# inhavl-shlee/AFI-GAN

Hardware: AMD Instinct MI355X
Metric: stage1_G+D_step_images_per_s (higher is better)
Workload: dtype f32 via f16x3: two scaled fp16 pieces per operand, three f16 MFMAs per product, fp32 accumulate (tensors fp32)

## Files before the change

### afigan_amd/csrc/afi_launch.h

```cpp
#pragma once
#include "afi_common.h"

int afi_launch_pix_gemm(const AfiPixGemm& p, int b_rc, hipStream_t st);
int afi_launch_gemm_tn(const float* Q, const float* V, float* dU, int planes, long long rows_per_plane, int M, int N, hipStream_t st, bool deterministic = false);
int afi_launch_gemm_nt(const float* A, const float* B, float* C, int planes, long long rows_per_plane, int N, int K, hipStream_t st);
int afi_launch_split_bf16_tiles(const float* B, void* out, int planes, int N, int K, int split, hipStream_t st);
int afi_launch_gemm_nt_bf16_dma(const float* A, const void* Bsplit, float* C, int planes, long long rows_per_plane, int N, int K, int split, hipStream_t st);
int afi_launch_gemm_tn_bf16(const float* Q, const float* V, float* dU, int planes, long long rows_per_plane, int M, int N, int split, hipStream_t st, bool deterministic = false);
int afi_launch_split_f16_tiles(const float* B, void* out, int planes, int N, int K, hipStream_t st, int wkind = 0);
int afi_f16_image_begin(void* out, hipStream_t st);
float* afi_f16_image_wmax(void* out);
long long afi_f16_image_bytes(int planes, int N, int K);
int afi_launch_absmax_planes(const float* X, long long per_plane, int planes, float* out, hipStream_t st);
AfiF16Bound afi_f16_bound(const float* amax, int kind);
int afi_launch_gemm_nt_f16x3(const float* A, const void* Bimg, float* C, int planes, long long rows_per_plane, int N, int K, const AfiF16Bound& ab, hipStream_t st,
                             bool a_pre = false, long long nt256_min_tiles = 512, bool local_sums = false);
int afi_launch_gemm_tn_f16x3(const float* Q, const float* V, float* dU, int planes, long long rows_per_plane, int M, int N, const AfiF16Bound& qb, const AfiF16Bound& vb,
                             hipStream_t st, bool pre = false, bool deterministic = false);
int afi_launch_wgrad_gemm(const AfiWgradGemm& p, hipStream_t st);
int afi_launch_wgrad_gemm_group(const AfiWgradGemm* probs, int n, int wide, hipStream_t st);
int afi_launch_wgrad_gemm_group6(const AfiWgradGemm* probs, int n, hipStream_t st);
int afi_launch_pix_gemm_group(const AfiPixGemm* probs, int n, int b_rc, hipStream_t st);

long long afi_wk6_image_bytes(int Ncols, int Ck, int ntaps, int nKphase);
int afi_launch_wk6_images(const AfiWk6ImgJob* jobs, int n, hipStream_t st, const AfiWk6Side* side = nullptr, const AfiWk6ConvT* ct = nullptr);
int afi_launch_pix_gemm_sk(const AfiPixGemm& p, int b_rc, hipStream_t st);
int afi_launch_pix_gemm_wk_group(const AfiPixGemm* probs, int n, int b_rc, hipStream_t st);
int afi_launch_wgrad_group(const AfiWgradGemm* probs, int n, int wide, hipStream_t st);
int afi_launch_wgrad6_group(const AfiWgradGemm* probs, int n, hipStream_t st);

int afi_launch_nchw_to_nhwc(const float* in, float* out, int N, int C, int P, hipStream_t st);
int afi_launch_cast_to_f32_nhwc(const void* in, int dt, int N, int C, int H, int W, long long sN, long long sC, long long sH, long long sW, float* out,
                                hipStream_t st);
int afi_launch_cast_from_f32_nhwc(const AfiView& in, int N, int H, int W, int C, void* out, int dt, hipStream_t st);

int afi_launch_colsum_group(const AfiColsumProb* probs, int n, hipStream_t st);
int afi_launch_nhwc_to_nchw(const float* in, float* out, int N, int C, int P, hipStream_t st);
int afi_launch_convT_pack(const float* W, float* Wp, int Cin, int Cout, hipStream_t st);
int afi_launch_convT_unpack_grad(const float* dWp, float* dW, int Cin, int Cout, hipStream_t st);
int afi_launch_rdb_wgrad_unpack(const float* dWp, float* const dw[4], int C, int G, float alpha, hipStream_t st);
int afi_launch_rdb_wgrad_unpack_multi(const float* dWp, long long stride, float* const (*dw)[4], int nblocks, int C, int G, float alpha, hipStream_t st);
int afi_launch_g_bwd_tail(const AfiColsumProb* cs, int n_cs, const float* dWpT, float* dWT, int Cin, int Cout,
                          const float* dWp, long long stride, float* const (*dw)[4], int nblocks, int C, int G, float alpha, hipStream_t st);
int afi_launch_rdb_xpart_pack(const float* const w[4], float* out, int C, int G, hipStream_t st);
int afi_launch_lrelu_slice(AfiView v, int N, int H, int W, int nch, hipStream_t st);
int afi_launch_bn_stats(const float* x, long long P, int C, float* mean, float* invstd, float* var_out, float* running_mean,
                        float* running_var, float* scratch, hipStream_t st, long long* num_batches_tracked = nullptr, float eps = -1.f,
                        float momentum = -1.f, bool fp64 = true);
int afi_launch_bn_stats_from_partials(const double* partial, int rows, long long P, int C, float* mean, float* invstd, float* var_out, float* running_mean,
                                      float* running_var, hipStream_t st, long long* num_batches_tracked = nullptr, float eps = -1.f, float momentum = -1.f);
int afi_launch_view_absmax(AfiView x, int N, int H, int W, int C, float* amax, hipStream_t st);
int afi_launch_bn_apply_lrelu(const float* x, float* y, const float* mean, const float* invstd, const float* gamma, const float* beta,
// ... 50 lines not shown
```

### afigan_amd/csrc/igemm.hip

```cpp
#include "afi_common.h"
#include "afi_launch.h"

#define AFI_BK 32
#define AFI_LDK (AFI_BK + 4)


__device__ __attribute__((aligned(16))) float afi_zeros[4] = {0.f, 0.f, 0.f, 0.f};

#include "afi_epilogue.h"

template <bool POST>
__global__ __launch_bounds__(256) void afi_pix_splitk_epilogue_kernel(const AfiPixGemm p) {
    const int HW = p.H * p.W;
    const long long M = (long long)p.N * HW;
    const int ldp = (p.Ncols + 3) & ~3;
    const int C_F4 = ldp >> 2;
    const long long total = M * C_F4;
    for (long long it = (long long)blockIdx.x * 256 + threadIdx.x; it < total; it += (long long)gridDim.x * 256) {
        const long long m = it / C_F4;
        const int col = (int)(it - m * C_F4) * 4;
        f32x4 v = {0.f, 0.f, 0.f, 0.f};
        const float* src = p.partial + m * ldp + col;
        const long long slab = M * ldp;
        int ks = 0;
// ... 509 lines not shown
#include <mutex>
namespace {
struct ProfRec { hipEvent_t a, b; int kind; double flops; long long m; int n, k, split, planes; };
struct ProfState {
    std::atomic<bool> on{false};
    std::mutex mu;
    std::vector<ProfRec> recs;
    std::vector<hipEvent_t> pool;
    size_t used = 0;
} g_prof;
const char* kKindNames[] = {
    "pix_gemm<128x128,KC,linear> (1x1 / ragged-map / non-aligned Winograd GEMMs)", "pix_gemm<128x64,KC>", "pix_gemm<128x32,KC>", "pix_gemm<64x64,KC>",
    "pix_gemm<128x128,RC,linear> (conv dgrad, mid-size / ragged maps)", "pix_gemm<128x64,RC>", "pix_gemm<128x32,RC>", "pix_gemm<64x64,RC>",
    "wgrad_gemm<128x128>", "wgrad_gemm<64x128>", "wgrad_gemm<32x128>",
    "pix_gemm<128x128,KC,halo> (conv fwd)", "pix_gemm<128x128,RC,halo> (conv dgrad)",
    "gemm_nt<128x128> (batched Winograd GEMM)", "gemm_tn<128x128> (Winograd weight-gradient GEMM)",
    "pix_gemm_wk (small-map pixel GEMM, K split inside the block; grouped launches included)",
    "wgrad_group (grouped weight gradients of a small-map backward pass)",
    "gemm_nt_bf16<128x128> (batched Winograd GEMM on the bf16 MFMA: bf16x6 / bf16x3 / bf16 operands, fp32 accumulate)",
    "gemm_tn_bf16<128x128> (Winograd weight-gradient GEMM on the bf16 MFMA: bf16x6 / bf16x3 / bf16 operands, fp32 accumulate)",
    "wgrad_group6 (grouped weight gradients of a small-map backward pass on the bf16 MFMA, bf16x6 operands, fp32 accumulate)",
    "pix_gemm_wk6 (small-map pixel GEMM on the bf16 MFMA, bf16x6 operands on pre-split weight images, fp32 accumulate; grouped launches included)",
    "gemm_nt_f16x3 (batched Winograd GEMM on the f16 MFMA, 256x256 tiles where the grid fills the chip and 128x128 below: two scaled fp16 pieces per operand, three products, fp32 accumulate)",
    "gemm_tn_f16x3<128x128> (Winograd weight-gradient GEMM on the f16 MFMA: two scaled fp16 pieces per operand, three products, fp32 accumulate)"};
constexpr int kNumKinds = 23;
hipEvent_t prof_event() {
    if (g_prof.used == g_prof.pool.size()) {
        hipEvent_t e;
        (void)hipEventCreate(&e);
        g_prof.pool.push_back(e);
    }
    return g_prof.pool[g_prof.used++];
}
struct ProfScope {
    hipStream_t st; int kind; double flops; hipEvent_t a{};
    long long m = 0; int n = 0, k = 0, split = 1, planes = 1;
    ProfScope(hipStream_t s, int kd, double f) : st(s), kind(kd), flops(f) {
        if (g_prof.on) { std::lock_guard<std::mutex> lk(g_prof.mu); a = prof_event(); (void)hipEventRecord(a, st); started = true; }
    }
    bool live = true, started = false;
    void cancel() { live = false; }
    ~ProfScope() {
        if (started && live) { std::lock_guard<std::mutex> lk(g_prof.mu); hipEvent_t b = prof_event(); (void)hipEventRecord(b, st); g_prof.recs.push_back({a, b, kind, flops, m, n, k, split, planes}); }
    }
};
}

extern "C" int afi_profile_enable(int on) {
    std::lock_guard<std::mutex> lk(g_prof.mu);
    if (on) { g_prof.recs.clear(); g_prof.used = 0; }
    g_prof.on = on != 0;
    return AFI_OK;
}
extern "C" int afi_profile_num_kinds(void) { return kNumKinds; }
extern "C" const char* afi_profile_kind_name(int kind) { return (kind >= 0 && kind < kNumKinds) ? kKindNames[kind] : ""; }
extern "C" int afi_profile_get(int kind, double* out) {
    out[0] = out[1] = out[2] = 0.0;
    for (const ProfRec& r : g_prof.recs) {
        if (r.kind != kind) continue;
        if (hipEventSynchronize(r.b) != hipSuccess) return AFI_ERR_LAUNCH;
        float ms = 0.f;
        if (hipEventElapsedTime(&ms, r.a, r.b) != hipSuccess) return AFI_ERR_LAUNCH;
        out[0] += 1.0; out[1] += ms; out[2] += r.flops;
    }
    return AFI_OK;
}

#include <stdio.h>
extern "C" int afi_profile_dump(const char* path) {
// ... 441 lines not shown
```

### afigan_amd/frozen.py

```python
import torch
import torch.nn as nn

from . import ops
from ._lib import AfiError

FROZEN_BN_EPS = 1e-5


class FrozenBatchNorm2d(nn.Module):

    def __init__(self, num_features, eps=FROZEN_BN_EPS):
        super().__init__()
        self.num_features, self.eps = num_features, eps
        self.register_buffer("weight", torch.ones(num_features))
        self.register_buffer("bias", torch.zeros(num_features))
        self.register_buffer("running_mean", torch.zeros(num_features))
        self.register_buffer("running_var", torch.ones(num_features) - eps)


def fold_conv(conv, norm=None, scale=1.0):
    w = conv.weight.detach().double()
    b = conv.bias.detach().double() if conv.bias is not None else torch.zeros(w.shape[0], dtype=torch.float64, device=w.device)
    if norm is not None:
        s = norm.weight.double() * torch.rsqrt(norm.running_var.double() + norm.eps)
# ... 2 lines not shown
    w, b = w.float(), (b * scale).float().contiguous()
    k = conv.kernel_size if isinstance(conv.kernel_size, int) else (conv.kernel_size[0] if len(set(conv.kernel_size)) == 1 else 0)
    if k == 1:
        return w.reshape(w.shape[0], w.shape[1]).contiguous(), b
    if k == 3:
        return ops.to_ohwi(w), b
    return w.contiguous(), b


class Conv2d(nn.Module):

    def __init__(self, cin, cout, k, stride=1, bias=False, norm=True):
        super().__init__()
        self.kernel_size, self.stride = k, stride
        w = torch.randn(cout, cin, k, k) * (2.0 / (cout * k * k)) ** 0.5
        self.weight = nn.Parameter(w, requires_grad=False)
        self.bias = nn.Parameter(torch.zeros(cout), requires_grad=False) if bias else None
        self.norm = FrozenBatchNorm2d(cout) if norm else None

    def fold(self, scale=1.0):
        return fold_conv(self, self.norm, scale)


def conv1x1(x, wb, stride=1, add=None, relu=False, alpha=1.0, add_scale=1.0):
    if stride != 1:
        x = x[:, :, ::stride, ::stride]
    if add is not None and add.shape[-2:] != x.shape[-2:]:
        raise AfiError(f"resnet_guide: addend {tuple(add.shape)} does not match the conv output {tuple(x.shape[-2:])}")
    return ops.conv1x1_fwd(x, wb[0], wb[1], add=add, add_scale=add_scale, alpha=alpha, act=2 if relu else 0)


def conv3x3(x, wb, stride=1, relu=False):
    act = 2 if relu else 0
    if stride == 2:
        return ops.conv3x3s2_fwd(x, wb[0], wb[1], act=act)
    N, C, H, W = x.shape
    if C >= 128 and wb[0].shape[0] >= 128 and N * H * W >= 1024:
        return ops.conv3x3_wino_infer(x, wb[0], wb[1], act=act)
    return ops.conv3x3_fwd(x, wb[0], wb[1], lrelu=act)


def prepared(module, name, tensors, build):
    key = tuple((t._version, t.data_ptr(), str(t.device)) for t in tensors)
    if getattr(module, f"_{name}_key", None) != key:
        setattr(module, f"_{name}", build())
        setattr(module, f"_{name}_key", key)
    return getattr(module, f"_{name}")


def adopt_prepared(module, name, tensors):
    if not hasattr(module, f"_{name}_key"):
        raise AfiError(f"adopt_prepared: {type(module).__name__} has no prepared slot {name!r} to adopt (prepared() builds it first)")
# ... 20 lines not shown
```

### afigan_amd/guide.py

```python
import math

import torch
import torch.nn as nn
import torch.nn.functional as F

from . import ops


def _kaiming(shape, fan_in, gain=1.0):
    return torch.randn(shape) * (gain * math.sqrt(2.0 / fan_in))


class _Conv1x1(nn.Module):
    def __init__(self, cin, cout, stride=1, relu=False, gain=1.0):
        super().__init__()
        self.stride, self.relu = stride, relu
        self.register_buffer("w", _kaiming((cin, cout), cin, gain).t().contiguous())
        self.register_buffer("b", torch.zeros(cout))

    def forward(self, x, add=None, relu=None):
        if self.stride != 1:
            x = x[:, :, ::self.stride, ::self.stride]
        return ops.conv1x1_fwd(x, self.w, self.b, add=add, act=2 if (self.relu if relu is None else relu) else 0)


class _Conv3x3(nn.Module):
    def __init__(self, cin, cout, relu=False):
        super().__init__()
        self.relu = relu
        self.register_buffer("w", _kaiming((cout, 3, 3, cin), cin * 9).permute(0, 3, 1, 2))
        self.register_buffer("b", torch.zeros(cout))

    def forward(self, x):
        N, C, H, W = x.shape
        if C >= 128 and self.w.shape[0] >= 128 and N * H * W >= 1024:
            return ops.conv3x3_wino_infer(x, self.w, self.b, act=2 if self.relu else 0)
        return ops.conv3x3_fwd(x, self.w, self.b, lrelu=2 if self.relu else 0)


class _Bottleneck(nn.Module):
    def __init__(self, cin, mid, cout, stride):
        super().__init__()
        self.c1 = _Conv1x1(cin, mid, stride, relu=True)
        self.c2 = _Conv3x3(mid, mid, relu=True)
        self.c3 = _Conv1x1(mid, cout, gain=0.25)
        self.short = _Conv1x1(cin, cout, stride) if (cin != cout or stride != 1) else None
# ... 6 lines not shown
class GuideR50FPN(nn.Module):

    def __init__(self, out_channels=256):
        super().__init__()
        self.register_buffer("stem_w", _kaiming((3 * 49, 64), 3 * 49))
        self.register_buffer("stem_b", torch.zeros(64))
        cfg = [(64, 64, 256, 3, 1), (256, 128, 512, 4, 2), (512, 256, 1024, 6, 2), (1024, 512, 2048, 3, 2)]
        self.stages = nn.ModuleList()
        for cin, mid, cout, n, stride in cfg:
            blocks = [_Bottleneck(cin, mid, cout, stride)] + [_Bottleneck(cout, mid, cout, 1) for _ in range(n - 1)]
            self.stages.append(nn.Sequential(*blocks))
        self.lateral = nn.ModuleList([_Conv1x1(c, out_channels, gain=0.1) for c in (256, 512, 1024, 2048)])
        self.output = nn.ModuleList([_Conv3x3(out_channels, out_channels) for _ in range(4)])
        self.register_buffer("pixel_mean", torch.tensor([103.53, 116.28, 123.675]).view(1, 3, 1, 1))
        self.eval()

    @torch.no_grad()
    def forward(self, images):
        x = (images - self.pixel_mean) * (1.0 / 58.0)
        H, W = x.shape[-2:]
        ph, pw = (32 - H % 32) % 32, (32 - W % 32) % 32
        if ph or pw:
            x = F.pad(x, (0, pw, 0, ph))
        N, _, H, W = x.shape
        cols = F.unfold(x, kernel_size=7, padding=3, stride=2)
        y = F.relu_(torch.baddbmm(self.stem_b.view(1, 1, -1), cols.transpose(1, 2), self.stem_w.unsqueeze(0).expand(N, -1, -1)))
        x = y.view(N, H // 2, W // 2, 64).permute(0, 3, 1, 2)
        x = F.max_pool2d(x, 3, 2, 1).contiguous(memory_format=torch.channels_last)
        feats = []
        for st in self.stages:
            x = st(x)
            feats.append(x)
        prev = self.lateral[3](feats[3])
        outs = [self.output[3](prev)]
        for i in (2, 1, 0):
            up = F.interpolate(prev, scale_factor=2, mode="nearest")
            prev = self.lateral[i](feats[i], add=up)
            outs.insert(0, self.output[i](prev))
        outs.append(outs[-1][:, :, ::2, ::2].contiguous(memory_format=torch.channels_last))
        return {f"p{i + 2}": o for i, o in enumerate(outs)}
```

### afigan_amd/ops.py

```python
import contextlib
import ctypes as C
import os

import numpy as np
import torch

from . import _lib
from ._lib import View, call

_NULL_VIEW = View(None, 0, 0, 0)


def stream_ptr():
    return C.c_void_p(torch.cuda.current_stream().cuda_stream)


def _check_cuda(*ts):
    for t in ts:
        if t is None:
            continue
        if not t.is_cuda:
            raise _lib.AfiError("the AFI-GAN hot path runs on the GPU only (got a CPU tensor); there is no CPU fallback")
        if t.dtype != torch.float32:
            raise _lib.AfiError(f"fp32 only on this path, got {t.dtype}")
# ... 372 lines not shown
        dw = new_ohwi(Cout, Cin, 3, 3, dy.device)
    assert dw.permute(0, 2, 3, 1).is_contiguous()
    call("afi_conv3x3s2_wgrad", view_of(dy), view_of(x), N, Hi, Wi, Cout, Cin, _p(dw), float(alpha), stream_ptr())
    return dw


def relu_bwd(g, act, scale=1.0):
    _check_cuda(g, act)
    assert is_dense_pm(g) and is_dense_pm(act) and g.shape == act.shape
    out = new_pixel_major(*g.shape, g.device)
    call("afi_relu_bwd", _p(g), _p(act), _p(out), g.numel(), float(scale), stream_ptr())
    return out


def conv1x1_fwd(x, w, bias=None, add=None, add_scale=1.0, alpha=1.0, out=None, act=0):
    _check_cuda(x, w, bias, add, out)
    _ensure_op_scratch(x.device)
    N, Cin, H, W = x.shape
    Cout = w.shape[0]
    w2 = w.reshape(Cout, Cin).contiguous()
    if out is None:
        out = new_pixel_major(N, Cout, H, W, x.device)
    call("afi_conv1x1_fwd", view_of(x), N, H, W, Cin, _p(w2), _p(bias), Cout, view_of(out), float(alpha), 0.0,
         view_of(add) if add is not None else _NULL_VIEW, float(add_scale), int(act), stream_ptr())
    return out


def conv1x1_dgrad(dy, w, dx=None, alpha=1.0, beta=0.0, out_dtype=torch.float32, *, z=None, z_act="lrelu", add=None, add_scale=1.0):
    _check_cuda(dy, w, dx, z, add)
    _ensure_op_scratch(dy.device)
    N, Cout, H, W = dy.shape
    Cin = w.shape[1]
    w2 = w.reshape(Cout, Cin).contiguous()
    if z is not None or add is not None:
        if out_dtype != torch.float32:
            raise _lib.AfiError("conv1x1_dgrad: z= / add= go with an fp32 dx")
        if dx is None:
            dx = new_pixel_major(N, Cin, H, W, dy.device)
        for name, t in (("dx", dx), ("z", z), ("add", add)):
            if t is not None and tuple(t.shape) != (N, Cin, H, W):
                raise _lib.AfiError(f"conv1x1_dgrad: {name} {tuple(t.shape)} is not the conv's input shape {(N, Cin, H, W)}")
        call("afi_conv1x1_dgrad_act", view_of(dy), N, H, W, Cout, _p(w2), Cin, view_of(dx), float(alpha), float(beta),
             view_of(add) if add is not None else _NULL_VIEW, float(add_scale), view_of(z) if z is not None else _NULL_VIEW,
             _z_act("conv1x1_dgrad", z, z_act) if z is not None else 0, stream_ptr())
        return dx
    if out_dtype != torch.float32:
# ... 1567 lines not shown
```

### afigan_amd/resnet_guide.py

```python
import torch
import torch.nn as nn

from . import _lib, ops, registry
from ._lib import AfiError
from .fpn_sr import ShapeSpec
from .frozen import FROZEN_BN_EPS, Conv2d, FrozenBatchNorm2d, adopt_prepared, cfg_get, check_forward_only, conv1x1, conv3x3, prepared
from .rpn import _wino

_BLOCKS = {50: [3, 4, 6, 3], 101: [3, 4, 23, 3]}


class _Frozen(nn.Module):
    what = "the ResNet-FPN guide"

    def _own_convs(self):
        raise NotImplementedError

    def _fold_own(self, convs):
        return {id(m): m.fold() for m in convs}

    def _prepare_tensors(self, convs):
        return [t for m in convs for t in list(m.parameters()) + list(m.buffers())]

    def _prepare(self):
        convs = self._own_convs()
        return prepared(self, "folded", self._prepare_tensors(convs), lambda: self._fold_own(convs))


class BasicStem(nn.Module):
    def __init__(self, in_channels=3, out_channels=64):
        super().__init__()
        self.conv1 = Conv2d(in_channels, out_channels, 7, stride=2)

    def run(self, x, f):
        return ops.resnet_stem(x, *f[id(self.conv1)])


class BottleneckBlock(nn.Module):

    def __init__(self, cin, cout, bottleneck, stride, stride_in_1x1):
        super().__init__()
        self.shortcut = Conv2d(cin, cout, 1, stride=stride) if cin != cout else None
        s1, s3 = (stride, 1) if stride_in_1x1 else (1, stride)
        self.conv1 = Conv2d(cin, bottleneck, 1, stride=s1)
        self.conv2 = Conv2d(bottleneck, bottleneck, 3, stride=s3)
        self.conv3 = Conv2d(bottleneck, cout, 1)

    def run(self, x, f):
        s = x if self.shortcut is None else conv1x1(x, f[id(self.shortcut)], self.shortcut.stride)
        y = conv1x1(x, f[id(self.conv1)], self.conv1.stride, relu=True)
        y = conv3x3(y, f[id(self.conv2)], self.conv2.stride, relu=True)
        return conv1x1(y, f[id(self.conv3)], add=s, relu=True)

    def convs(self):
        return [self.conv1, self.conv2, self.conv3] + ([self.shortcut] if self.shortcut is not None else [])

    def run_keep(self, x, f):
        s = x if self.shortcut is None else conv1x1(x, f[id(self.shortcut)], self.shortcut.stride)
        a1 = conv1x1(x, f[id(self.conv1)], self.conv1.stride, relu=True)
        a2 = conv3x3(a1, f[id(self.conv2)], self.conv2.stride, relu=True)
        return a1, a2, conv1x1(a2, f[id(self.conv3)], add=s, relu=True)


def _strided(t, stride):
    return t if stride == 1 else t[:, :, ::stride, ::stride]


def _dense_pm(t, like):
    if t is None:
        return None
    t = ops.pixel_major(t.float())
    if not ops.is_dense_pm(t):
        d = ops.new_pixel_major(*like.shape, like.device)
        d.copy_(t)
        t = d
# ... 123 lines not shown
    def _build(self, out_features, stem, stem_channels, counts, res2_out_channels, width, block):
        self._out_features = list(out_features)
        self.stem = stem
        self._out_feature_channels, self._out_feature_strides = {"stem": stem_channels}, {"stem": 4}
        cin, cout = stem_channels, res2_out_channels
        self.stage_names = []
        for i, n in enumerate(counts):
            name, first = f"res{i + 2}", (1 if i == 0 else 2)
            blocks = [block(i + 2, cin if j == 0 else cout, cout, width, first if j == 0 else 1) for j in range(n)]
            self.add_module(name, nn.Sequential(*blocks))
            self.stage_names.append(name)
            self._out_feature_channels[name], self._out_feature_strides[name] = cout, 4 * 2 ** i
            cin, cout, width = cout, 2 * cout, 2 * width

    @property
    def size_divisibility(self):
        return 0

    def output_shape(self):
        return {n: ShapeSpec(channels=self._out_feature_channels[n], stride=self._out_feature_strides[n]) for n in self._out_features}

    _train_stages = ()
    _fuse_masks = True

    def _wants_graph(self):
        return bool(self._train_stages) and torch.is_grad_enabled() and any(p.requires_grad for p in self.parameters())

    def forward(self, x):
        if self._wants_graph():
            return self._forward_train(x)
        check_forward_only(self, x, self.what)
        with torch.no_grad():
            f = self._prepare()
            out = {}
            y = self.stem.run(x.float(), f)
            if "stem" in self._out_features:
                out["stem"] = y
            for name in self.stage_names:
                for blk in getattr(self, name):
                    y = blk.run(y, f)
                if name in self._out_features:
                    out[name] = y
        return out


class ResNet(ResNetBase):

    def __init__(self, depth=50, out_features=("res2", "res3", "res4", "res5"), stride_in_1x1=True, width_per_group=64,
                 res2_out_channels=256, stem_out_channels=64):
        super().__init__()
        if depth not in _BLOCKS:
            raise AfiError(f"resnet_guide: RESNETS.DEPTH {depth} is not supported (50 or 101)")
        if stem_out_channels != 64:
            raise AfiError(f"resnet_guide: RESNETS.STEM_OUT_CHANNELS {stem_out_channels} is not supported (the stem kernel makes 64)")
        n_stages = self._num_stages("resnet_guide", out_features)
        if (width_per_group % 4) or (res2_out_channels % 4):
            raise AfiError("resnet_guide: channel counts must be multiples of 4")
        self._build(out_features, BasicStem(3, 64), 64, _BLOCKS[depth][:n_stages], res2_out_channels, width_per_group,
                    lambda stage, cin, cout, width, stride: BottleneckBlock(cin, cout, width, stride, stride_in_1x1))

    def _own_convs(self):
        return [m for m in self.modules() if isinstance(m, Conv2d)]

    def trainable_(self, freeze_at=2, fuse_masks=True):
        if freeze_at is False:
            stages = []
        else:
            if isinstance(freeze_at, bool) or not isinstance(freeze_at, int) or not 0 <= freeze_at <= 5:
                raise AfiError(f"resnet_guide: trainable_(freeze_at={freeze_at!r}): an integer 1..5 (BACKBONE.FREEZE_AT), or False to freeze everything")
# ... 101 lines not shown
    @property
    def size_divisibility(self):
        return self._size_divisibility

    def output_shape(self):
        return {n: ShapeSpec(channels=self._out_feature_channels[n], stride=self._out_feature_strides[n]) for n in self._out_features}

    def _own_convs(self):
        return self.lateral_convs + self.output_convs

    def _fold_own(self, convs):
        f = super()._fold_own(convs)
        if self._fuse_type == "avg":
            for m in self.lateral_convs[1:]:
                f[("avg", id(m))] = m.fold(scale=0.5)
        return f

    def forward(self, x):
        check_forward_only(self, x, self.what)
        feats = self.bottom_up(x)
        with torch.no_grad():
            f = self._prepare()
            xs = [feats[k] for k in self.in_features[::-1]]
            prev = conv1x1(xs[0], f[id(self.lateral_convs[0])])
            results = [conv3x3(prev, f[id(self.output_convs[0])])]
            for feat, lat, out in zip(xs[1:], self.lateral_convs[1:], self.output_convs[1:]):
                td = ops.nearest(prev, up=2)
                if self._fuse_type == "avg":
                    prev = conv1x1(feat, f[("avg", id(lat))], add=td, alpha=0.5, add_scale=0.5)
                else:
                    prev = conv1x1(feat, f[id(lat)], add=td)
                results.insert(0, conv3x3(prev, f[id(out)]))
            results.append(ops.nearest(results[-1], up=1, down=2))
        return dict(zip(self._out_features, results))


def _resnet_from_cfg(cfg, input_shape=None):
    r = cfg_get(cfg.MODEL, "RESNETS", None)
    if input_shape is not None and getattr(input_shape, "channels", 3) not in (None, 3):
        raise AfiError(f"resnet_guide: 3 input channels only, got {input_shape.channels}")
    norm = cfg_get(r, "NORM", "FrozenBN")
    if norm != "FrozenBN":
        raise AfiError(f"resnet_guide: RESNETS.NORM {norm!r} is not supported (the frozen guide folds FrozenBN)")
    if cfg_get(r, "NUM_GROUPS", 1) != 1:
        raise AfiError(f"resnet_guide: RESNETS.NUM_GROUPS {cfg_get(r, 'NUM_GROUPS', 1)} is not supported (groups = 1 only)")
    if cfg_get(r, "RES5_DILATION", 1) != 1:
        raise AfiError(f"resnet_guide: RESNETS.RES5_DILATION {cfg_get(r, 'RES5_DILATION', 1)} is not supported (no dilation)")
    if any(cfg_get(r, "DEFORM_ON_PER_STAGE", [False] * 4)):
        raise AfiError("resnet_guide: deformable convolutions (RESNETS.DEFORM_ON_PER_STAGE) are not supported")
    if cfg_get(r, "RADIX", 1) != 1 or cfg_get(r, "DEEP_STEM", False) or cfg_get(r, "AVD", False) or cfg_get(r, "AVG_DOWN", False):
        raise AfiError("resnet_guide: the ResNeSt options (RESNETS.RADIX / DEEP_STEM / AVD / AVG_DOWN) are not supported")
    return ResNet(depth=cfg_get(r, "DEPTH", 50), out_features=list(cfg_get(r, "OUT_FEATURES", ["res4"])),
                  stride_in_1x1=bool(cfg_get(r, "STRIDE_IN_1X1", True)), width_per_group=cfg_get(r, "WIDTH_PER_GROUP", 64),
                  res2_out_channels=cfg_get(r, "RES2_OUT_CHANNELS", 256), stem_out_channels=cfg_get(r, "STEM_OUT_CHANNELS", 64))
# ... 24 lines not shown
```

### include/afigan_hip.h

```cpp
#ifndef AFIGAN_HIP_H
#define AFIGAN_HIP_H

#include <stddef.h>
#include <stdint.h>

#ifdef __cplusplus
extern "C" {
#endif

#define AFI_OK 0
#define AFI_ERR_BAD_ARG 1
#define AFI_ERR_UNSUPPORTED 2
#define AFI_ERR_LAUNCH 3
#define AFI_ERR_WORKSPACE 4

#define AFI_MAX_RDB 8

typedef struct afi_view {
    float* p;
    long long sN, sH, sW;
} afi_view_t;

int afi_abi_version(void);
const char* afi_status_string(int status);
// ... 198 lines not shown
} afi_det_sgd_desc_t;
long long afi_detector_sgd_units(long long n, int O, int I, int k, int fold);
int afi_detector_sgd_step(const afi_det_sgd_desc_t* descs_host, const afi_det_sgd_desc_t* descs_dev, int ntensors, long long max_units,
                          const int* unit_off_dev, long long total_units, float momentum, float gscale, void* stream);

int afi_nchw_to_nhwc(const float* in, float* out, int N, int C, int P, void* stream);
int afi_nhwc_to_nchw(const float* in, float* out, int N, int C, int P, void* stream);
int afi_cast_to_f32_nhwc(const void* src, int src_dtype, int N, int C, int H, int W, long long sN, long long sC, long long sH, long long sW,
                         float* dst, void* stream);
int afi_cast_from_f32_nhwc(afi_view_t src, int N, int H, int W, int C, void* dst, int dst_dtype, void* stream);

long long afi_resize_bilinear_u8_ws_bytes(int H0, int W0, int C, int H1, int W1);
int afi_resize_bilinear_u8(const unsigned char* src, int H0, int W0, int C, unsigned char* dst, int H1, int W1, int hflip,
                           int out_chw, void* ws, long long ws_bytes, void* stream);
long long afi_dual_scale_u8_ws_bytes(int H0, int W0, int C, int H1, int W1, int H2, int W2);
int afi_dual_scale_u8(const unsigned char* src, int H0, int W0, int C, unsigned char* image, int H1, int W1, int hflip,
                      unsigned char* image_r, int H2, int W2, int hflip_r, int out_chw, void* ws, long long ws_bytes, void* stream);
int afi_normalize_pad_u8(const unsigned char* img_chw, int C, int H, int W, const float* mean, const float* std_,
                         float* out, int Hp, int Wp, void* stream);

int afi_resnet_stem_fwd(const float* x, int N, int H, int W, const float* w, const float* bias, float* out, void* stream);
int afi_nearest_nhwc(afi_view_t x, int N, int H, int W, int C, int up, int down, float* out, void* stream);

#define AFI_POOL_MAX3S2P1 0
#define AFI_POOL_AVG3S2P1 1
#define AFI_POOL_AVG2S2_CEIL 2
int afi_resnest_stem_fwd(const float* x, int N, int H, int W, const float* w, const float* bias, int Cout, float* out, void* stream);
int afi_resnest_pool_nhwc(afi_view_t x, int N, int H, int W, int C, int mode, float* out, void* stream);
long long afi_resnest_splat_ws_floats(int N, int H, int W, int C);
int afi_resnest_splat_gap(afi_view_t s0, afi_view_t s1, int N, int H, int W, int C, float* part, long long part_floats, void* stream);
int afi_resnest_splat_attn(const float* part, int N, int H, int W, int C, int I, const float* w1, const float* b1, const float* w2,
                           const float* b2, float* att, void* stream);
int afi_resnest_splat_combine(afi_view_t s0, afi_view_t s1, int N, int H, int W, int C, const float* att, int avd, float* out, void* stream);

int afi_resnest_splat_attn_keep(const float* part, int N, int H, int W, int C, int I, const float* w1, const float* b1, const float* w2,
                                const float* b2, float* att, float* g, float* h, void* stream);
long long afi_resnest_splat_bwd_ws_floats(int N, int H, int W, int C);
int afi_resnest_splat_bwd_dots(afi_view_t dout, afi_view_t s0, afi_view_t s1, int N, int H, int W, int C, int avd, float* part,
                               long long part_floats, void* stream);
int afi_resnest_splat_bwd_attn(const float* part, int N, int H, int W, int C, int I, const float* att, const float* h, const float* w1,
                               const float* w2, float* dz, float* dh, float* dg, void* stream);
int afi_resnest_splat_bwd_params(const float* dz, const float* dh, const float* g, const float* h, const float* s1, int N, int C, int I,
                                 float* dw1, float* db1, float* dw2, float* db2, void* stream);
int afi_resnest_splat_bwd_combine(afi_view_t dout, afi_view_t s0, afi_view_t s1, int N, int H, int W, int C, const float* att, const float* dg,
                                  int avd, afi_view_t ds0, afi_view_t ds1, void* stream);
int afi_resnest_pool_bwd(const float* dy, int N, int H, int W, int C, int mode, afi_view_t dx, float beta, afi_view_t z_or_null, void* stream);
// ... 154 lines not shown
```

Before: 29.15.

## Add frozen-weight 1x1 conv kernel with cached pre-split bf16 weight images

Adds a dedicated forward 1x1 convolution kernel for frozen (no-grad) weights in the ResNet guide and FPN laterals. The weights are split into bf16 fragments once and cached per module, so each call only splits activations, into LDS, and runs six bf16 MFMA products with a fused bias, residual add and activation epilogue. The guide stem also switches from unfold+baddbmm to the existing native stem kernel. This aims to cut per-call weight splitting and generic GEMM overhead, at the cost of a new code path and cached images that must be invalidated when parameters change.

Result: faster. 29.75, median of 6 (+2.1%).

```diff
diff --git a/afigan_amd/csrc/afi_launch.h b/afigan_amd/csrc/afi_launch.h
--- a/afigan_amd/csrc/afi_launch.h
+++ b/afigan_amd/csrc/afi_launch.h
@@ -21,6 +21,8 @@
 int afi_launch_wgrad_gemm_group(const AfiWgradGemm* probs, int n, int wide, hipStream_t st);
 int afi_launch_wgrad_gemm_group6(const AfiWgradGemm* probs, int n, hipStream_t st);
 int afi_launch_pix_gemm_group(const AfiPixGemm* probs, int n, int b_rc, hipStream_t st);
+void* afi_prof_open(hipStream_t st, int kind, double flops, long long m, int n, int k);
+void afi_prof_close(void* scope);
 
 long long afi_wk6_image_bytes(int Ncols, int Ck, int ntaps, int nKphase);
 int afi_launch_wk6_images(const AfiWk6ImgJob* jobs, int n, hipStream_t st, const AfiWk6Side* side = nullptr, const AfiWk6ConvT* ct = nullptr);
@@ -28,6 +30,9 @@
 int afi_launch_pix_gemm_wk_group(const AfiPixGemm* probs, int n, int b_rc, hipStream_t st);
 int afi_launch_wgrad_group(const AfiWgradGemm* probs, int n, int wide, hipStream_t st);
 int afi_launch_wgrad6_group(const AfiWgradGemm* probs, int n, hipStream_t st);
+
+#define AFI_FROZEN1X1_PLAN_SLOTS 12
+enum { AFI_F1_M = 0, AFI_F1_BM, AFI_F1_BN, AFI_F1_KC, AFI_F1_NTM, AFI_F1_NTN, AFI_F1_GRID, AFI_F1_LDS, AFI_F1_XBYTES, AFI_F1_OBYTES, AFI_F1_IBYTES, AFI_F1_XDENSE };
 
 int afi_launch_nchw_to_nhwc(const float* in, float* out, int N, int C, int P, hipStream_t st);
 int afi_launch_cast_to_f32_nhwc(const void* in, int dt, int N, int C, int H, int W, long long sN, long long sC, long long sH, long long sW, float* out,
diff --git a/afigan_amd/csrc/frozen1x1.hip b/afigan_amd/csrc/frozen1x1.hip
--- /dev/null
+++ b/afigan_amd/csrc/frozen1x1.hip
@@ -0,0 +1,235 @@
+#include "afi_common.h"
+#include "afi_launch.h"
+#include "afi_bf16_split.h"
+
+#define AFI_F1_ROWS 64
+struct AfiFrozen1x1 {
+    const float* x; long long x_sN, x_sH, x_sW;
+    const unsigned char* image; const float* bias; const float* add; float* out;
+    unsigned x_bytes, o_bytes, i_bytes;
+    int x_dense, M, HW, W, Cin, Cout, kc, ntile_n, nst;
+    float alpha, add_scale; int act;
+};
+
+__device__ __forceinline__ int afi_f1_logical_id() {
+    const int nwg = gridDim.x, qq = nwg >> 3, rr = nwg & 7, xcd = blockIdx.x & 7;
+    return (xcd < rr ? xcd * (qq + 1) : rr * (qq + 1) + (xcd - rr) * qq) + (int)(blockIdx.x >> 3);
+}
+
+template <int NJ>
+__global__ __launch_bounds__(256, 2) void afi_frozen1x1_kernel(const AfiFrozen1x1 p) {
+    extern __shared__ __attribute__((aligned(16))) unsigned char lds[];
+    const int tid = threadIdx.x, lane = tid & 63, l15 = lane & 15, lq = lane >> 4;
+    const int wave = __builtin_amdgcn_readfirstlane(tid >> 6);
+    const int lb = afi_f1_logical_id();
+    const int tile_m = lb / p.ntile_n, tile_n = lb - tile_m * p.ntile_n;
+    const int m0 = tile_m * AFI_F1_ROWS;
+    const int kc = p.kc, nks = kc >> 5, nchunks = p.Cin / kc, part_bytes = kc * 128;
+    const int pl = kc == 128 ? 5 : (kc == 64 ? 4 : 3);
+    const int iters = 1 << (pl - 2);
+    const __amdgpu_buffer_rsrc_t rsrc_x = __builtin_amdgcn_make_buffer_rsrc((void*)p.x, 0, p.x_bytes, 0x00020000);
+    const __amdgpu_buffer_rsrc_t rsrc_b = __builtin_amdgcn_make_buffer_rsrc((void*)p.image, 0, p.i_bytes, 0x00020000);
+
+    const int q = tid & ((1 << pl) - 1), r0 = tid >> pl, rstep = 256 >> pl;
+    unsigned row_off[8];
+#pragma unroll
+    for (int i = 0; i < 8; ++i) {
+        const int m = m0 + r0 + i * rstep;
+        unsigned off = 0xFFFFFFFFu;
+        if (i < iters && m < p.M) {
+            if (p.x_dense) off = 4u * (unsigned)m * (unsigned)p.x_sW;
+            else {
+                const int img = m / p.HW, rem = m - img * p.HW, y = rem / p.W, xx = rem - y * p.W;
+                off = 4u * (unsigned)(img * p.x_sN + y * p.x_sH + xx * p.x_sW);
+            }
+        }
+        row_off[i] = off;
+    }
+    u32x4 a_raw[8];
+    auto load_chunk = [&](int c) {
+#pragma unroll
+        for (int i = 0; i < 8; ++i)
+            if (i < iters)
+                a_raw[i] = __builtin_amdgcn_raw_buffer_load_b128(rsrc_x, row_off[i] == 0xFFFFFFFFu ? 0xFFFFFFFFu : row_off[i] + (unsigned)(4 * (c * kc) + 16 * q), 0, 0);
+    };
+    const int s_ks = q >> 3, s_lq = (q >> 1) & 3, s_half = q & 1;
+    auto split_store = [&]() {
+#pragma unroll
+        for (int i = 0; i < 8; ++i)
+            if (i < iters) {
+                const int row = r0 + i * rstep, mi = row >> 4, rl = row & 15;
+                const f32x4 v = __builtin_bit_cast(f32x4, a_raw[i]);
+                unsigned h0, m0_, l0, h1, m1_, l1;
+                afi_split3_pair(v[0], v[1], h0, m0_, l0);
+                afi_split3_pair(v[2], v[3], h1, m1_, l1);
+                unsigned char* d = lds + ((s_ks * 4 + mi) * 64 + 16 * s_lq + (rl ^ (4 * s_lq))) * 16 + 8 * s_half;
+                *(u32x2*)d = u32x2{h0, h1};
+                *(u32x2*)(d + part_bytes) = u32x2{m0_, m1_};
+                *(u32x2*)(d + 2 * part_bytes) = u32x2{l0, l1};
+            }
+    };
+
+    const int h0 = (tile_n * 4 + wave) * NJ;
+    const int frag_off = 16 * (16 * lq + (l15 ^ (4 * lq)));
+    u32x4 bq[3];
+    auto load_b = [&](int j, int stage) {
+        int h = h0 + j;
+        if (h * 16 >= p.Cout) h = 0;
+        const int st = stage < p.nst ? stage : p.nst - 1;
+        const int soff = ((h >> 1) * p.nst + st) * AFI_WK6_STAGE_BYTES + 3 * (h & 1) * 1024;
+#pragma unroll
+        for (int pt = 0; pt < 3; ++pt) bq[pt] = __builtin_amdgcn_raw_buffer_load_b128(rsrc_b, (unsigned)(16 * lane + pt * 1024), soff, 0);
+    };
+    f32x4 acc[NJ][4];
+#pragma unroll
+    for (int j = 0; j < NJ; ++j)
+#pragma unroll
+        for (int mi = 0; mi < 4; ++mi) acc[j][mi] = f32x4{0.f, 0.f, 0.f, 0.f};
+    auto mfma = [](u32x4 wf, u32x4 xf, f32x4 c) -> f32x4 {
+        return __builtin_amdgcn_mfma_f32_16x16x32_bf16(__builtin_bit_cast(bf16x8, wf), __builtin_bit_cast(bf16x8, xf), c, 0, 0, 0);
+    };
+
+    load_chunk(0);
+    load_b(0, 0);
+    for (int c = 0; c < nchunks; ++c) {
+        split_store();
+        __syncthreads();
+        if (c + 1 < nchunks) load_chunk(c + 1);
+        for (int ks = 0; ks < nks; ++ks) {
+            u32x4 fa[4][3];
+#pragma unroll
+            for (int mi = 0; mi < 4; ++mi)
+#pragma unroll
+                for (int pt = 0; pt < 3; ++pt) fa[mi][pt] = *(const u32x4*)(lds + pt * part_bytes + (ks * 4 + mi) * 1024 + frag_off);
+            const int stage = c * nks + ks;
+#pragma unroll
+            for (int j = 0; j < NJ; ++j) {
+                const u32x4 bh = bq[0], bm = bq[1], bl = bq[2];
+                if (j + 1 < NJ) load_b(j + 1, stage); else load_b(0, stage + 1);
+#pragma unroll
+                for (int mi = 0; mi < 4; ++mi) acc[j][mi] = mfma(bh, fa[mi][2], acc[j][mi]);
+#pragma unroll
+                for (int mi = 0; mi < 4; ++mi) acc[j][mi] = mfma(bl, fa[mi][0], acc[j][mi]);
+#pragma unroll
+                for (int mi = 0; mi < 4; ++mi) acc[j][mi] = mfma(bm, fa[mi][1], acc[j][mi]);
+#pragma unroll
+                for (int mi = 0; mi < 4; ++mi) acc[j][mi] = mfma(bh, fa[mi][1], acc[j][mi]);
+#pragma unroll
+                for (int mi = 0; mi < 4; ++mi) acc[j][mi] = mfma(bm, fa[mi][0], acc[j][mi]);
+#pragma unroll
+                for (int mi = 0; mi < 4; ++mi) acc[j][mi] = mfma(bh, fa[mi][0], acc[j][mi]);
+            }
+        }
+        if (c + 1 < nchunks) __syncthreads();
+    }
+
+    const __amdgpu_buffer_rsrc_t rsrc_o = __builtin_amdgcn_make_buffer_rsrc((void*)p.out, 0, p.o_bytes, 0x00020000);
+    const __amdgpu_buffer_rsrc_t rsrc_r = __builtin_amdgcn_make_buffer_rsrc((void*)p.add, 0, p.add ? p.o_bytes : 0u, 0x00020000);
+    const float slope = p.act == 1 ? AFI_LRELU_SLOPE : 0.f;
+#pragma unroll
+    for (int j = 0; j < NJ; ++j) {
+        const int col = 16 * (h0 + j) + 4 * lq;
+        if (16 * (h0 + j) >= p.Cout) break;
+        f32x4 bias = {0.f, 0.f, 0.f, 0.f};
+        if (p.bias) bias = *(const f32x4*)(p.bias + col);
+        unsigned off[4];
+        f32x4 r[4];
+#pragma unroll
+        for (int mi = 0; mi < 4; ++mi) {
+            const int m = m0 + 16 * mi + l15;
+            off[mi] = m < p.M ? 4u * ((unsigned)m * (unsigned)p.Cout + (unsigned)col) : 0xFFFFFFFFu;
+            r[mi] = f32x4{0.f, 0.f, 0.f, 0.f};
+            if (p.add) r[mi] = __builtin_bit_cast(f32x4, __builtin_amdgcn_raw_buffer_load_b128(rsrc_r, off[mi], 0, 0));
+        }
+#pragma unroll
+        for (int mi = 0; mi < 4; ++mi) {
+            f32x4 v = p.alpha * acc[j][mi];
+            v += bias;
+            if (p.add) v += p.add_scale * r[mi];
+            if (p.act) {
+#pragma unroll
+                for (int e = 0; e < 4; ++e) v[e] = v[e] > 0.f ? v[e] : v[e] * slope;
+            }
+            __builtin_amdgcn_raw_buffer_store_b128(__builtin_bit_cast(u32x4, v), rsrc_o, off[mi], 0, 0);
+        }
+    }
+}
+
+extern "C" int afi_frozen1x1_plan(int N, int H, int W, int Cin, int Cout, long long x_sN, long long x_sH, long long x_sW, long long o_sN, long long o_sH,
+                                  long long o_sW, int has_add, long long a_sN, long long a_sH, long long a_sW, long long* plan) {
+    if (!plan || N <= 0 || H <= 0 || W <= 0 || Cin <= 0 || Cout <= 0) return AFI_ERR_BAD_ARG;
+    for (int i = 0; i < AFI_FROZEN1X1_PLAN_SLOTS; ++i) plan[i] = 0;
+    if ((Cin & 31) || (Cout & 31)) return AFI_ERR_UNSUPPORTED;
+    const long long kLimit = 0x7FFFFFF0LL;
+    const long long M = (long long)N * H * W;
+    if (M > (1LL << 30)) return AFI_ERR_UNSUPPORTED;
+    if (x_sW < Cin || x_sW % Cin != 0) return AFI_ERR_UNSUPPORTED;
+    const long long s = x_sW / Cin, row_span = ((long long)(W - 1) * s + 1) * Cin;
+    if (H > 1 && x_sH < s * row_span) return AFI_ERR_UNSUPPORTED;
+    if (N > 1 && x_sN < (long long)(H - 1) * x_sH + row_span) return AFI_ERR_UNSUPPORTED;
+    if ((x_sN | x_sH | x_sW) & 3) return AFI_ERR_UNSUPPORTED;
+    if (x_sN < 0 || x_sH < 0) return AFI_ERR_UNSUPPORTED;
+    const long long x_elems = (long long)(N - 1) * x_sN + (long long)(H - 1) * x_sH + (long long)(W - 1) * x_sW + Cin;
+    if (x_elems * 4 >= kLimit) return AFI_ERR_UNSUPPORTED;
+    if (o_sW != Cout || o_sH != (long long)W * Cout || o_sN != (long long)H * W * Cout) return AFI_ERR_UNSUPPORTED;
+    if (has_add && (a_sW != o_sW || a_sH != o_sH || a_sN != o_sN)) return AFI_ERR_UNSUPPORTED;
+    const long long o_bytes = M * Cout * 4;
+    if (o_bytes >= kLimit) return AFI_ERR_UNSUPPORTED;
+    const long long i_bytes = afi_wk6_image_bytes(Cout, Cin, 1, 1);
+    if (i_bytes >= kLimit) return AFI_ERR_UNSUPPORTED;
+    const bool dense = x_sH == (long long)W * x_sW && x_sN == (long long)H * x_sH;
+    const long long ntm = (M + AFI_F1_ROWS - 1) / AFI_F1_ROWS;
+    int bn = 64;
+    for (int cand = 256; cand > 64; cand >>= 1) {
+        if (cand > ((Cout + 63) & ~63)) continue;
+        if (ntm * ((Cout + cand - 1) / cand) >= 512) { bn = cand; break; }
+    }
+    const long long ntn = (Cout + bn - 1) / bn;
+    if (ntm * ntn > 0x3FFFFFFFLL) return AFI_ERR_UNSUPPORTED;
+    const int kc = (Cin % 128 == 0) ? 128 : ((Cin % 64 == 0) ? 64 : 32);
+    plan[AFI_F1_M] = M; plan[AFI_F1_BM] = AFI_F1_ROWS; plan[AFI_F1_BN] = bn; plan[AFI_F1_KC] = kc;
+    plan[AFI_F1_NTM] = ntm; plan[AFI_F1_NTN] = ntn; plan[AFI_F1_GRID] = ntm * ntn; plan[AFI_F1_LDS] = 3LL * AFI_F1_ROWS * kc * 2;
+    plan[AFI_F1_XBYTES] = x_elems * 4; plan[AFI_F1_OBYTES] = o_bytes; plan[AFI_F1_IBYTES] = i_bytes; plan[AFI_F1_XDENSE] = dense ? 1 : 0;
+    return AFI_OK;
+}
+
+extern "C" long long afi_frozen1x1_image_bytes(int Cout, int Cin) {
+    if (Cout <= 0 || Cin <= 0 || (Cout & 31) || (Cin & 31)) return 0;
+    return afi_wk6_image_bytes(Cout, Cin, 1, 1);
+}
+
+extern "C" int afi_conv1x1_frozen_image(afi_ctx_t* ctx, const float* w, int Cout, int Cin, void* image, long long image_bytes, void* stream) {
+    (void)ctx;
+    if (!w || !image || Cout <= 0 || Cin <= 0) return AFI_ERR_BAD_ARG;
+    if ((Cout & 31) || (Cin & 31)) return AFI_ERR_UNSUPPORTED;
+    if (image_bytes < afi_wk6_image_bytes(Cout, Cin, 1, 1)) return AFI_ERR_WORKSPACE;
+    const AfiWk6ImgJob job = {w, (long long)Cin, 0, Cout, Cin, 1, 1, 0, (unsigned char*)image};
+    return afi_launch_wk6_images(&job, 1, (hipStream_t)stream);
+}
+
+extern "C" int afi_conv1x1_frozen_fwd(afi_ctx_t* ctx, afi_view_t x, int N, int H, int W, int Cin, const void* image, const float* bias, int Cout, afi_view_t out,
+                                      float alpha, afi_view_t add, float add_scale, int act, void* stream) {
+    (void)ctx;
+    if (!x.p || !out.p || !image || act < 0 || act > 2) return AFI_ERR_BAD_ARG;
+    long long plan[AFI_FROZEN1X1_PLAN_SLOTS];
+    AFI_TRY(afi_frozen1x1_plan(N, H, W, Cin, Cout, x.sN, x.sH, x.sW, out.sN, out.sH, out.sW, add.p != nullptr, add.sN, add.sH, add.sW, plan));
+    if ((((uintptr_t)x.p | (uintptr_t)out.p | (uintptr_t)image | (uintptr_t)add.p | (uintptr_t)bias) & 15)) return AFI_ERR_UNSUPPORTED;
+    AfiFrozen1x1 p;
+    p.x = x.p; p.x_sN = x.sN; p.x_sH = x.sH; p.x_sW = x.sW;
+    p.image = (const unsigned char*)image; p.bias = bias; p.add = add.p; p.out = out.p;
+    p.x_bytes = (unsigned)plan[AFI_F1_XBYTES]; p.o_bytes = (unsigned)plan[AFI_F1_OBYTES]; p.i_bytes = (unsigned)plan[AFI_F1_IBYTES];
+    p.x_dense = (int)plan[AFI_F1_XDENSE]; p.M = (int)plan[AFI_F1_M]; p.HW = H * W; p.W = W; p.Cin = Cin; p.Cout = Cout;
+    p.kc = (int)plan[AFI_F1_KC]; p.ntile_n = (int)plan[AFI_F1_NTN]; p.nst = Cin / 32;
+    p.alpha = alpha; p.add_scale = add_scale; p.act = act;
+    const hipStream_t st = (hipStream_t)stream;
+    const dim3 grid((unsigned)plan[AFI_F1_GRID]), block(256);
+    const unsigned lds = (unsigned)plan[AFI_F1_LDS];
+    void* prof = afi_prof_open(st, 23, 2.0 * (double)p.M * Cin * Cout, p.M, Cout, Cin);
+    switch ((int)plan[AFI_F1_BN]) {
+        case 256: hipLaunchKernelGGL(afi_frozen1x1_kernel<4>, grid, block, lds, st, p); break;
+        case 128: hipLaunchKernelGGL(afi_frozen1x1_kernel<2>, grid, block, lds, st, p); break;
+        default:  hipLaunchKernelGGL(afi_frozen1x1_kernel<1>, grid, block, lds, st, p); break;
+    }
+    afi_prof_close(prof);
+    return hipGetLastError() == hipSuccess ? AFI_OK : AFI_ERR_LAUNCH;
+}
diff --git a/afigan_amd/csrc/igemm.hip b/afigan_amd/csrc/igemm.hip
--- a/afigan_amd/csrc/igemm.hip
+++ b/afigan_amd/csrc/igemm.hip
@@ -555,8 +555,9 @@
     "wgrad_group6 (grouped weight gradients of a small-map backward pass on the bf16 MFMA, bf16x6 operands, fp32 accumulate)",
     "pix_gemm_wk6 (small-map pixel GEMM on the bf16 MFMA, bf16x6 operands on pre-split weight images, fp32 accumulate; grouped launches included)",
     "gemm_nt_f16x3 (batched Winograd GEMM on the f16 MFMA, 256x256 tiles where the grid fills the chip and 128x128 below: two scaled fp16 pieces per operand, three products, fp32 accumulate)",
-    "gemm_tn_f16x3<128x128> (Winograd weight-gradient GEMM on the f16 MFMA: two scaled fp16 pieces per operand, three products, fp32 accumulate)"};
-constexpr int kNumKinds = 23;
+    "gemm_tn_f16x3<128x128> (Winograd weight-gradient GEMM on the f16 MFMA: two scaled fp16 pieces per operand, three products, fp32 accumulate)",
+    "frozen1x1 (forward 1x1 conv of frozen weights on the bf16 MFMA: bf16x6 operands, weights pre-split into a fragment image built once, fp32 accumulate)"};
+constexpr int kNumKinds = 24;
 hipEvent_t prof_event() {
     if (g_prof.used == g_prof.pool.size()) {
         hipEvent_t e;
@@ -578,6 +579,13 @@
     }
 };
 }
+void* afi_prof_open(hipStream_t st, int kind, double flops, long long m, int n, int k) {
+    if (!g_prof.on) return nullptr;
+    ProfScope* s = new ProfScope(st, kind, flops);
+    s->m = m; s->n = n; s->k = k;
+    return s;
+}
+void afi_prof_close(void* scope) { delete (ProfScope*)scope; }
 
 extern "C" int afi_profile_enable(int on) {
     std::lock_guard<std::mutex> lk(g_prof.mu);
diff --git a/afigan_amd/frozen.py b/afigan_amd/frozen.py
--- a/afigan_amd/frozen.py
+++ b/afigan_amd/frozen.py
@@ -48,12 +48,19 @@
         return fold_conv(self, self.norm, scale)
 
 
-def conv1x1(x, wb, stride=1, add=None, relu=False, alpha=1.0, add_scale=1.0):
+def conv1x1(x, wb, stride=1, add=None, relu=False, alpha=1.0, add_scale=1.0, owner=None):
     if stride != 1:
         x = x[:, :, ::stride, ::stride]
     if add is not None and add.shape[-2:] != x.shape[-2:]:
         raise AfiError(f"resnet_guide: addend {tuple(add.shape)} does not match the conv output {tuple(x.shape[-2:])}")
+    if owner is not None and ops.conv1x1_frozen_routed(x, wb[0].shape[0], add):
+        return ops.conv1x1_frozen_fwd(x, conv1x1_image(owner, wb[0]), wb[1], wb[0].shape[0], add=add, add_scale=add_scale, alpha=alpha,
+                                      act=2 if relu else 0)
     return ops.conv1x1_fwd(x, wb[0], wb[1], add=add, add_scale=add_scale, alpha=alpha, act=2 if relu else 0)
+
+
+def conv1x1_image(module, w, name="image1x1"):
+    return prepared(module, name, list(module.parameters()) + list(module.buffers()), lambda: ops.conv1x1_frozen_image(w))
 
 
 def conv3x3(x, wb, stride=1, relu=False):
diff --git a/afigan_amd/guide.py b/afigan_amd/guide.py
--- a/afigan_amd/guide.py
+++ b/afigan_amd/guide.py
@@ -4,7 +4,7 @@
 import torch.nn as nn
 import torch.nn.functional as F
 
-from . import ops
+from . import frozen, ops
 
 
 def _kaiming(shape, fan_in, gain=1.0):
@@ -21,7 +21,10 @@
     def forward(self, x, add=None, relu=None):
         if self.stride != 1:
             x = x[:, :, ::self.stride, ::self.stride]
-        return ops.conv1x1_fwd(x, self.w, self.b, add=add, act=2 if (self.relu if relu is None else relu) else 0)
+        act = 2 if (self.relu if relu is None else relu) else 0
+        if ops.conv1x1_frozen_routed(x, self.w.shape[0], add):
+            return ops.conv1x1_frozen_fwd(x, frozen.conv1x1_image(self, self.w), self.b, self.w.shape[0], add=add, act=act)
+        return ops.conv1x1_fwd(x, self.w, self.b, add=add, act=act)
 
 
 class _Conv3x3(nn.Module):
@@ -74,11 +77,8 @@
         ph, pw = (32 - H % 32) % 32, (32 - W % 32) % 32
         if ph or pw:
             x = F.pad(x, (0, pw, 0, ph))
-        N, _, H, W = x.shape
-        cols = F.unfold(x, kernel_size=7, padding=3, stride=2)
-        y = F.relu_(torch.baddbmm(self.stem_b.view(1, 1, -1), cols.transpose(1, 2), self.stem_w.unsqueeze(0).expand(N, -1, -1)))
-        x = y.view(N, H // 2, W // 2, 64).permute(0, 3, 1, 2)
-        x = F.max_pool2d(x, 3, 2, 1).contiguous(memory_format=torch.channels_last)
+        w7 = frozen.prepared(self, "stem_w7", [self.stem_w], lambda: self.stem_w.t().reshape(64, 3, 7, 7).contiguous())
+        x = ops.resnet_stem(x, w7, self.stem_b)
         feats = []
         for st in self.stages:
             x = st(x)
diff --git a/afigan_amd/ops.py b/afigan_amd/ops.py
--- a/afigan_amd/ops.py
+++ b/afigan_amd/ops.py
@@ -418,6 +418,58 @@
     if out is None:
         out = new_pixel_major(N, Cout, H, W, x.device)
     call("afi_conv1x1_fwd", view_of(x), N, H, W, Cin, _p(w2), _p(bias), Cout, view_of(out), float(alpha), 0.0,
+         view_of(add) if add is not None else _NULL_VIEW, float(add_scale), int(act), stream_ptr())
+    return out
+
+
+FROZEN1X1_MIN_PIXELS = 8192
+FROZEN1X1_MIN_PIXELS_EXPANDING = 2048
+frozen1x1_route = True
+frozen1x1_images_built = 0
+_F1_PLAN = ("M", "BM", "BN", "KC", "ntile_m", "ntile_n", "grid", "lds_bytes", "x_bytes", "out_bytes", "image_bytes", "x_dense")
+
+
+def conv1x1_frozen_plan(N, H, W, Cin, Cout, x_strides, out_strides=None, add_strides=None):
+    o = out_strides if out_strides is not None else (H * W * Cout, W * Cout, Cout)
+    a = add_strides if add_strides is not None else (0, 0, 0)
+    plan = (C.c_longlong * len(_F1_PLAN))()
+    st = _lib.load().afi_frozen1x1_plan(N, H, W, Cin, Cout, *[int(s) for s in x_strides], *[int(s) for s in o], int(add_strides is not None),
+                                        *[int(s) for s in a], plan)
+    if st == _lib.DEFINES["AFI_ERR_UNSUPPORTED"]:
+        return None
+    _lib.check(st, "afi_frozen1x1_plan")
+    return dict(zip(_F1_PLAN, plan))
+
+
+def conv1x1_frozen_routed(x, Cout, add=None):
+    N, Cin, H, W = x.shape
+    least = min(FROZEN1X1_MIN_PIXELS, FROZEN1X1_MIN_PIXELS_EXPANDING) if Cout >= 2 * Cin else FROZEN1X1_MIN_PIXELS
+    if not frozen1x1_route or N * H * W < least or x.stride(1) != 1 or (add is not None and not is_dense_pm(add)):
+        return False
+    return conv1x1_frozen_plan(N, H, W, Cin, Cout, (x.stride(0), x.stride(2), x.stride(3)),
+                               add_strides=(add.stride(0), add.stride(2), add.stride(3)) if add is not None else None) is not None
+
+
+def conv1x1_frozen_image(w):
+    global frozen1x1_images_built
+    _check_cuda(w)
+    Cout, Cin = w.shape[0], w.shape[1]
+    w2 = w.reshape(Cout, Cin).contiguous()
+    nbytes = _lib.load().afi_frozen1x1_image_bytes(Cout, Cin)
+    if nbytes <= 0:
+        raise _lib.AfiError(f"conv1x1_frozen_image: Cout {Cout} and Cin {Cin} must be positive multiples of 32")
+    image = torch.empty(nbytes, device=w.device, dtype=torch.uint8)
+    call("afi_conv1x1_frozen_image", _p(w2), Cout, Cin, _p(image), nbytes, stream_ptr())
+    frozen1x1_images_built += 1
+    return image
+
+
+def conv1x1_frozen_fwd(x, image, bias, Cout, add=None, add_scale=1.0, alpha=1.0, out=None, act=0):
+    _check_cuda(x, bias, add, out)
+    N, Cin, H, W = x.shape
+    if out is None:
+        out = new_pixel_major(N, Cout, H, W, x.device)
+    call("afi_conv1x1_frozen_fwd", view_of(x), N, H, W, Cin, _p(image), _p(bias), Cout, view_of(out), float(alpha),
          view_of(add) if add is not None else _NULL_VIEW, float(add_scale), int(act), stream_ptr())
     return out
 
diff --git a/afigan_amd/resnet_guide.py b/afigan_amd/resnet_guide.py
--- a/afigan_amd/resnet_guide.py
+++ b/afigan_amd/resnet_guide.py
@@ -46,11 +46,12 @@
         self.conv2 = Conv2d(bottleneck, bottleneck, 3, stride=s3)
         self.conv3 = Conv2d(bottleneck, cout, 1)
 
-    def run(self, x, f):
-        s = x if self.shortcut is None else conv1x1(x, f[id(self.shortcut)], self.shortcut.stride)
-        y = conv1x1(x, f[id(self.conv1)], self.conv1.stride, relu=True)
+    def run(self, x, f, route=False):
+        own = (lambda m: m) if route else (lambda m: None)
+        s = x if self.shortcut is None else conv1x1(x, f[id(self.shortcut)], self.shortcut.stride, owner=own(self.shortcut))
+        y = conv1x1(x, f[id(self.conv1)], self.conv1.stride, relu=True, owner=own(self.conv1))
         y = conv3x3(y, f[id(self.conv2)], self.conv2.stride, relu=True)
-        return conv1x1(y, f[id(self.conv3)], add=s, relu=True)
+        return conv1x1(y, f[id(self.conv3)], add=s, relu=True, owner=own(self.conv3))
 
     def convs(self):
         return [self.conv1, self.conv2, self.conv3] + ([self.shortcut] if self.shortcut is not None else [])
@@ -220,6 +221,7 @@
 
     _train_stages = ()
     _fuse_masks = True
+    _route_frozen1x1 = False
 
     def _wants_graph(self):
         return bool(self._train_stages) and torch.is_grad_enabled() and any(p.requires_grad for p in self.parameters())
@@ -236,13 +238,14 @@
                 out["stem"] = y
             for name in self.stage_names:
                 for blk in getattr(self, name):
-                    y = blk.run(y, f)
+                    y = blk.run(y, f, route=True) if self._route_frozen1x1 else blk.run(y, f)
                 if name in self._out_features:
                     out[name] = y
         return out
 
 
 class ResNet(ResNetBase):
+    _route_frozen1x1 = True
 
     def __init__(self, depth=50, out_features=("res2", "res3", "res4", "res5"), stride_in_1x1=True, width_per_group=64,
                  res2_out_channels=256, stem_out_channels=64):
@@ -390,14 +393,15 @@
         with torch.no_grad():
             f = self._prepare()
             xs = [feats[k] for k in self.in_features[::-1]]
-            prev = conv1x1(xs[0], f[id(self.lateral_convs[0])])
+            own = (lambda m: m) if getattr(self.bottom_up, "_route_frozen1x1", False) else (lambda m: None)
+            prev = conv1x1(xs[0], f[id(self.lateral_convs[0])], owner=own(self.lateral_convs[0]))
             results = [conv3x3(prev, f[id(self.output_convs[0])])]
             for feat, lat, out in zip(xs[1:], self.lateral_convs[1:], self.output_convs[1:]):
                 td = ops.nearest(prev, up=2)
                 if self._fuse_type == "avg":
-                    prev = conv1x1(feat, f[("avg", id(lat))], add=td, alpha=0.5, add_scale=0.5)
+                    prev = conv1x1(feat, f[("avg", id(lat))], add=td, alpha=0.5, add_scale=0.5, owner=own(lat))
                 else:
-                    prev = conv1x1(feat, f[id(lat)], add=td)
+                    prev = conv1x1(feat, f[id(lat)], add=td, owner=own(lat))
                 results.insert(0, conv3x3(prev, f[id(out)]))
             results.append(ops.nearest(results[-1], up=1, down=2))
         return dict(zip(self._out_features, results))
diff --git a/include/afigan_hip.h b/include/afigan_hip.h
--- a/include/afigan_hip.h
+++ b/include/afigan_hip.h
@@ -244,6 +244,13 @@
 int afi_resnet_stem_fwd(const float* x, int N, int H, int W, const float* w, const float* bias, float* out, void* stream);
 int afi_nearest_nhwc(afi_view_t x, int N, int H, int W, int C, int up, int down, float* out, void* stream);
 
+long long afi_frozen1x1_image_bytes(int Cout, int Cin);
+int afi_frozen1x1_plan(int N, int H, int W, int Cin, int Cout, long long x_sN, long long x_sH, long long x_sW, long long o_sN, long long o_sH,
+                       long long o_sW, int has_add, long long a_sN, long long a_sH, long long a_sW, long long* plan);
+int afi_conv1x1_frozen_image(afi_ctx_t* ctx, const float* w, int Cout, int Cin, void* image, long long image_bytes, void* stream);
+int afi_conv1x1_frozen_fwd(afi_ctx_t* ctx, afi_view_t x, int N, int H, int W, int Cin, const void* image, const float* bias, int Cout, afi_view_t out,
+                           float alpha, afi_view_t add_or_null, float add_scale, int act, void* stream);
+
 #define AFI_POOL_MAX3S2P1 0
 #define AFI_POOL_AVG3S2P1 1
 #define AFI_POOL_AVG2S2_CEIL 2
```
